# skitzoid/Box2D-MT

Hardware: AMD Instinct MI355X
Metric: world steps/sec at 99858 bodies per GPU (BASELINE config 3: Tumbler 100k, CCD off; Step = collide + island solve + broad-phase + state read-back); for N > 1: container-steps/s = world steps/s x N containers in the one sharded world (higher is better)
Workload: dtype f32

## Files before the change

box2d-mt_amd/csrc/b2d_kernels_collide.h:

```cpp
#ifndef B2D_KERNELS_COLLIDE_H
#define B2D_KERNELS_COLLIDE_H

#include "b2d_world.h"
#include "b2d_toi.h"
#include "b2d_scan.h"

__device__ __forceinline__ Xf loadXf(const float4* b_xf, int body)
{
	float4 t = b_xf[body];
	Xf xf;
	xf.p = v2(t.x, t.y);
	xf.q.s = t.z;
	xf.q.c = t.w;
	return xf;
}

__device__ __forceinline__ AABB loadAabb(const float4* p_fat, int proxy)
{
	float4 t = p_fat[proxy];
	AABB a;
	a.lo = v2(t.x, t.y);
	a.hi = v2(t.z, t.w);
	return a;
}
// ... 390 lines not shown
		c.cellExtBits = 0;
		c.gridFresh = 0;
		W.st->dbgCensus[0] = 0;
		c.nEvents = 0;
		c.nToiList = 0;
		c.nNewToiCand = 0;
		c.nToiEvents = 0;
		c.nToiCalls = 0;
		c.toiBase = 0;
		c.toiOverflow = 0;
		c.nToiLog = 0;
		c.toiIncomplete = 0;
		c.toiUnsafe = 0;
		c.nToiGroups = 0;
		c.nToiMoved = 0;
		c.nToiNewPairs = 0;
		c.nToiChainCreated = 0;
		c.nPreSolve = 0;
		c.nPostSolve = 0;
		c.nFilterList = 0;
		c.spToiCreated = 0;
		c.spToiStraddle = 0;
	}
	if (t < 32) bar[t] = t == 6 ? W.testSpinMax : 0;
	for (int k = t; k < ARRIVE_SITES * TREE_WORDS; k += (int)blockDim.x) W.arriveTree[k] = 0ull;
}

__global__ __launch_bounds__(256) void k_wake_apply(DW W)
{
	b2dPhaseStamp(W);
	for (int i = blockIdx.x * blockDim.x + threadIdx.x; i < W.nBodies; i += gridDim.x * blockDim.x)
	{
		if (W.b_wake[i])
		{
			W.b_flags[i] |= BF_AWAKE;
			W.b_pos[i].w = 0.0f;
			W.b_wake[i] = 0;
		}
	}
}

__global__ __launch_bounds__(256) void k_flag_filter(DW W, const unsigned long long* pairs, int nPairs)
{
	b2dPhaseStamp(W);
	DState* S = W.st;
	const int n = S->c.nContacts;
// ... 198 lines not shown
```

box2d-mt_amd/csrc/b2d_kernels_solve_large.h:

```cpp
#ifndef B2D_KERNELS_SOLVE_LARGE_H
#define B2D_KERNELS_SOLVE_LARGE_H

#include "b2d_kernels_solve_small.h"

#define LC_WORDS ((int)(sizeof(ContactConstraint) / 4))
#define LC_VEL_WORDS 36
#define LC_IMP_FIRST 10
#define LC_MASS_FIRST 28
#define LC_POS_FIRST 36

__device__ __forceinline__ void lcStore(const DW& W, int row, const ContactConstraint& cc, int first, int last)
{
	uint32_t words[LC_WORDS];
	memcpy(words, &cc, sizeof(ContactConstraint));
	uint32_t* dst = (uint32_t*)W.lc;
#pragma unroll
	for (int f = 0; f < LC_WORDS; ++f)
	{
		if (f >= first && f < last) dst[(size_t)f * W.capContacts + row] = words[f];
	}
}

__device__ __forceinline__ void lcLoad(const DW& W, int row, ContactConstraint& cc, int first, int last)
{
// ... 1622 lines not shown
			W.b_vel[body] = make_float4(vv.x, vv.y, w, 0.0f);
		}
	}
	{
		const int n = S->c.nLIslands;
		for (int k = blockIdx.x * blockDim.x + threadIdx.x; k < n; k += gridDim.x * blockDim.x)
		{
			W.rootPen[W.li_roots[k]] = 0;
			W.rootJointOkay[W.li_roots[k]] = 1;
		}
	}
	if (blockIdx.x == 0 && threadIdx.x == 0) S->c.allLargeDone = 0;
}

__global__ __launch_bounds__(256) void k_large_position(DW W, int color)
{
	asm volatile("" :: "s"(W.capContacts), "s"(color), "s"((unsigned long long)(uintptr_t)W.colorStart), "s"((unsigned long long)(uintptr_t)W.st),
		"s"((unsigned long long)(uintptr_t)W.li_ref), "s"((unsigned long long)(uintptr_t)W.lc), "s"((unsigned long long)(uintptr_t)W.b_pos),
		"s"((unsigned long long)(uintptr_t)W.rootDone), "s"((unsigned long long)(uintptr_t)W.rootPen), "s"((unsigned)blockDim.x), "s"((unsigned)gridDim.x), "s"(W.stampMask));
	b2dPhaseStamp(W);
	DState* S = W.st;
	const int allDone = S->c.allLargeDone;
	const int begin = W.colorStart[color], end = W.colorStart[color + 1];
	if (allDone) return;
	const ContactArrays& C = W.ca[S->cur];
	BlockMaxU32 pen;
	pen.key = -1; pen.val = 0u;
	for (int base = begin + blockIdx.x * blockDim.x; base < end; base += gridDim.x * blockDim.x)
	{
		const int row = base + threadIdx.x;
		bool valid = row < end;
		LargeRef r;
		r.root = 0;
		if (valid)
		{
			r = largeRef(W, C, row);
			valid = W.rootDone[r.root] == 0;
		}
		float minSep = 0.0f;
		if (valid)
		{
			ContactConstraint cc;
			memset(&cc, 0, sizeof(cc));
			lcLoad(W, row, cc, LC_MASS_FIRST, LC_MASS_FIRST + 4);
			lcLoad(W, row, cc, LC_POS_FIRST, LC_WORDS);
			float4 pa = W.b_pos[r.bodyA], pb = W.b_pos[r.bodyB];
			BodyPos pA, pB;
			pA.c = v2(pa.x, pa.y); pA.a = pa.z;
			pB.c = v2(pb.x, pb.y); pB.a = pb.z;
			b2dSolvePosition(&cc, &pA, &pB, B2D_BAUMGARTE, &minSep);
			if (r.nsA) W.b_pos[r.bodyA] = make_float4(pA.c.x, pA.c.y, pA.a, pa.w);
			if (r.nsB) W.b_pos[r.bodyB] = make_float4(pB.c.x, pB.c.y, pB.a, pb.w);
		}
		blockMaxU32Offer(pen, W.rootPen, r.root, floatBits(0.0f - minSep), valid);
	}
	blockMaxU32Flush(pen, W.rootPen);
}

__global__ __launch_bounds__(256) void k_large_pos_end(DW W)
{
	b2dPhaseStamp(W);
	DState* S = W.st;
	if (S->c.allLargeDone) return;
	__shared__ int s_open;
	if (threadIdx.x == 0) s_open = 0;
	__syncthreads();
	const int n = S->c.nLIslands;
	int open = 0;
	for (int k = threadIdx.x; k < n; k += blockDim.x)
// ... 85 lines not shown
```

box2d-mt_amd/csrc/b2d_kernels_sweep_end.h:

```cpp
#ifndef B2D_KERNELS_SWEEP_END_H
#define B2D_KERNELS_SWEEP_END_H

#include "b2d_handover.h"

#define SWEEP_END_LANES 512
#define SWEEP_END_WAVES (SWEEP_END_LANES / 64)
#define SE_HUB 1
#define SE_GUESS 2
#define SE_JOINTS_INIT 4
#define SE_JOINTS_VEL 8
#define SE_JOINTS_POS 16
#define SE_POS_END 32
#define SE_POS_BEGIN 64
#define SE_HUB_WIDE_ONLY 128

#define REST_ROWS_MAX 196608
#define REST_SERIAL_BIT (1ull << HUB_COLOR)
template <int MODE>
__device__ __forceinline__ bool restSweepRows(const DW& W, int restFirst, int nColors, int* bar, int epoch, int wg, int nWG, bool serialTagged)
{
	DState* S = W.st;
	const ContactArrays& C = W.ca[S->cur];
	const int begin = W.colorStart[restFirst], end = W.colorStart[nColors];
	const int tag = (epoch & 0x7fff) << 16;
// ... 628 lines not shown
	}
}

__global__ __launch_bounds__(256) void k_solver_recover_reset(DW W, int* bar)
{
	b2dPhaseStamp(W);
	DState* S = W.st;
	for (int i = blockIdx.x * blockDim.x + threadIdx.x; i < W.nBodies; i += gridDim.x * blockDim.x)
	{
		for (int k = 0; k < ROOT_PEN_SLOTS; ++k) W.rootPen[(size_t)k * W.nBodies + i] = 0;
		W.rootDone[i] = 0;
		W.rootSleepMin[i] = 0x7f7fffffu;
		W.rootJointOkay[i] = 1;
		W.bodyRest[i] = 0;
		W.bodyActive[i] = 0;
	}
	for (int i = blockIdx.x * blockDim.x + threadIdx.x; i < MAX_BLOCKS + 1; i += gridDim.x * blockDim.x)
	{
		W.blkCursor[(size_t)i * BLK_SLOT] = 0;
		W.blkBodyCursor[(size_t)i * BLK_SLOT] = 0;
	}
	if (blockIdx.x == 0 && threadIdx.x <= MAX_COLORS) W.colorCursor[colorSlot(threadIdx.x)] = 0;
	if (blockIdx.x == 0 && threadIdx.x < 32) bar[threadIdx.x] = 0;
	if (blockIdx.x == 0 && threadIdx.x == 0)
	{
		atomicAnd(&S->c.overflow, ~(64 | 0x2000));
		S->c.allLargeDone = 0;
		S->c.posItersLarge = 0;
	}
}

#endif
```

box2d-mt_amd/csrc/b2d_world.h:

```cpp
#ifndef B2D_WORLD_H
#define B2D_WORLD_H

#include "b2d_solver.h"
#include "b2d_joint.h"
#include "b2d_wave.h"

#define BF_TYPE_MASK 0x3u
#define BF_AWAKE 0x4u
#define BF_AUTOSLEEP 0x8u
#define BF_BULLET 0x10u
#define BF_FIXEDROT 0x20u
#define BF_ACTIVE 0x40u
#define BF_ISLAND 0x80u
#define BF_LARGE 0x100u

#define BT_STATIC 0u
#define BT_KINEMATIC 1u
#define BT_DYNAMIC 2u

#define CF_TOUCHING 0x1u
#define CF_ENABLED 0x2u
#define CF_FILTER 0x4u
#define CF_TOI_CANDIDATE 0x8u
#define CF_SENSOR 0x10u
// ... 438 lines not shown
{
	if (c.nBlocks == 0 || c.nOrphanRows > 0 || c.blkMaxRows > c.blkLanes || c.blkMaxBodies > c.blkLanes || c.nSerialOrphans > 2048) return false;
	if (c.partitionAge > 240 && (4 * c.nCutRows > c.nLContacts || 2 * c.nLContacts < 900)) return false;
	return true;
}

__device__ __forceinline__ void b2dStoreAgentI(int* p, int v) { __hip_atomic_store(p, v, __ATOMIC_RELAXED, __HIP_MEMORY_SCOPE_AGENT); }
__device__ __forceinline__ int b2dLoadAgentI(const int* p) { return __hip_atomic_load(p, __ATOMIC_RELAXED, __HIP_MEMORY_SCOPE_AGENT); }
__device__ __forceinline__ void b2dStoreAgent4(float4* p, float4 v)
{
	typedef float f4 __attribute__((ext_vector_type(4)));
	f4 q;
	q.x = v.x; q.y = v.y; q.z = v.z; q.w = v.w;
	asm volatile("global_store_dwordx4 %0, %1, off sc1\n\ts_nop 1" :: "v"(p), "v"(q) : "memory");
}
__device__ __forceinline__ float4 b2dLoadAgent4(const float4* p)
{
	typedef float f4 __attribute__((ext_vector_type(4)));
	f4 r;
	asm volatile("global_load_dwordx4 %0, %1, off sc1\n\ts_waitcnt vmcnt(0)" : "=v"(r) : "v"(p) : "memory");
	return make_float4(r.x, r.y, r.z, r.w);
}
#define TREE_GROUPS 32
#define TREE_STRIDE 16
#define TREE_WORDS ((TREE_GROUPS + 1) * TREE_STRIDE)
#define TREE_SUM_MAX 0xffffffu
#define ARRIVE_COLLIDE 0
#define ARRIVE_COMPACT 1
#define ARRIVE_EDGES 2
#define ARRIVE_CHAINS 3
#define ARRIVE_END_STEP 4
#define ARRIVE_CLASSIFY 5
#define ARRIVE_TOI_FIRST 6
#define ARRIVE_COLOR_CHECK 7
#define ARRIVE_PAIRS 8
#define ARRIVE_KEYSET 9
#define ARRIVE_SITES 10
__device__ __forceinline__ bool b2dTreeArrive(unsigned long long* tree, unsigned v0, unsigned v1, unsigned* t0, unsigned* t1)
{
	const unsigned nb = gridDim.x;
	const unsigned groups = nb < TREE_GROUPS ? nb : TREE_GROUPS;
	const unsigned g = blockIdx.x % groups;
	const unsigned members = nb / groups + (g < nb % groups ? 1u : 0u);
	const unsigned long long one = 1ull << 48;
	unsigned long long* slot = tree + (size_t)g * TREE_STRIDE;
	const unsigned long long add = one | ((unsigned long long)(v1 & TREE_SUM_MAX) << 24) | (unsigned long long)(v0 & TREE_SUM_MAX);
// ... 95 lines not shown
```

box2d-mt_amd/csrc/b2hip.hip:

```cpp
#include <hip/hip_runtime.h>

#include <math.h>
#include <stdio.h>
#include <stdlib.h>
#include <string.h>

#include <algorithm>
#include <dlfcn.h>
#include <rccl/rccl.h>
#include <atomic>
#include <chrono>
#include <thread>
#include <map>
#include <mutex>
#include <string>
#include <vector>

#include "../../include/b2hip.h"
#include "b2d_kernels_toi_chains.h"
#include "b2d_kernels_toi_domains.h"
#include "b2d_handover.h"
#include "b2d_kernels_solve_blocks.h"
#include "b2d_kernels_sweep_end.h"
#include "b2d_kernels_edit.h"
#include "b2d_kernels_shard.h"
#include "b2d_kernels_spatial.h"
#include "b2d_kernels_query.h"
#include "b2d_scan.h"
#include "b2d_shape_geom.h"

#include "b2hip_host_world.h"
#include "b2hip_host_phases.h"
#include "b2hip_host_toi.h"

extern "C"
{
#include "b2hip_api_world.h"
#include "b2hip_api_step.h"
#include "b2hip_api_snapshot.h"
#include "b2hip_api_sharding.h"
#include "b2hip_api_callbacks.h"
#include "b2hip_api_query.h"
}
```

box2d-mt_amd/csrc/b2hip_api_world.h:

```cpp


const char* b2hip_last_error(void)
{
	return g_lastError.c_str();
}

const char* b2hip_version(void)
{
	return "b2hip 0.1 (gfx950)";
}

int b2hip_world_create(const b2hip_world_def* def, b2hip_world** out)
{
	if (!def || !out) return setError(B2HIP_ERR_INVALID, "null argument");
	int count = 0;
	hipError_t e = hipGetDeviceCount(&count);
	if (e != hipSuccess || count <= 0)
	{
		return setError(B2HIP_ERR_NO_DEVICE, "no HIP device available: the b2hip Step() path has no CPU fallback");
	}
	int current = 0;
	if (hipGetDevice(&current) != hipSuccess) current = 0;
	const int device = def->device >= 0 ? def->device : current;
	if (device >= count) return setError(B2HIP_ERR_NO_DEVICE, "no such HIP device");
// ... 59 lines not shown
				hipOccupancyMaxActiveBlocksPerMultiprocessor(&perCU2, k_solve_blocks<512>, 512, 0) == hipSuccess &&
				hipOccupancyMaxActiveBlocksPerMultiprocessor(&perCU3, k_solve_blocks<BLOCK_LANES>, BLOCK_LANES, 0) == hipSuccess &&
				perCU > 0 && perCU2 > 0 && perCU3 > 0)
			{
				w->blocksMaxWG = prop.multiProcessorCount - 8;
				int s0 = 0, s1 = 0, s2 = 0;
				if (hipOccupancyMaxActiveBlocksPerMultiprocessor(&s0, k_blocks_sweep<256>, 256, 0) == hipSuccess &&
					hipOccupancyMaxActiveBlocksPerMultiprocessor(&s1, k_blocks_sweep<512>, 512, 0) == hipSuccess &&
					hipOccupancyMaxActiveBlocksPerMultiprocessor(&s2, k_blocks_sweep<BLOCK_LANES>, BLOCK_LANES, 0) == hipSuccess)
				{
					w->sweepMaxWG[0] = std::max(1, s0 - 1) * w->blocksMaxWG;
					w->sweepMaxWG[1] = std::max(1, s1 - 1) * w->blocksMaxWG;
					w->sweepMaxWG[2] = std::max(1, s2 - 1) * w->blocksMaxWG;
				}
			}
			int r1 = 0, r2 = 0, f1 = 0, f2 = 0;
			const int cus = std::max(1, prop.multiProcessorCount - 8);
			if (hipOccupancyMaxActiveBlocksPerMultiprocessor(&r1, k_large_rest<1>, 256, 0) == hipSuccess &&
				hipOccupancyMaxActiveBlocksPerMultiprocessor(&r2, k_large_rest<2>, 256, 0) == hipSuccess && r1 > 0 && r2 > 0)
				w->restMaxWG = std::min(r1, r2) * cus;
			if (hipOccupancyMaxActiveBlocksPerMultiprocessor(&f1, k_rest_hub<1>, SWEEP_END_LANES, 0) == hipSuccess &&
				hipOccupancyMaxActiveBlocksPerMultiprocessor(&f2, k_rest_hub<2>, SWEEP_END_LANES, 0) == hipSuccess && f1 > 0 && f2 > 0)
				w->restHubMaxWG = std::min(f1, f2) * cus;
		}
	}
	w->dfEpoch = 0;
	for (int i = 0; i < 13; ++i) w->ev[i] = nullptr;
	w->h_dstate = nullptr;
	for (int i = 0; i < 13; ++i)
	{
		if (hipEventCreate(&w->ev[i]) != hipSuccess)
		{
			b2hip_world_destroy(w);
			return setError(B2HIP_ERR_HIP, "hipEventCreate failed");
		}
	}
	if (hipHostMalloc((void**)&w->h_dstate, sizeof(DState), hipHostMallocDefault) != hipSuccess)
	{
		b2hip_world_destroy(w);
		return setError(B2HIP_ERR_HIP, "hipHostMalloc failed");
	}
	if (hipHostMalloc((void**)&w->h_pub, sizeof(DState), hipHostMallocMapped | hipHostMallocCoherent) != hipSuccess ||
		hipHostGetDevicePointer((void**)&w->d_pub, w->h_pub, 0) != hipSuccess)
	{
		b2hip_world_destroy(w);
		return setError(B2HIP_ERR_HIP, "hipHostMalloc (coherent) failed");
// ... 697 lines not shown
	StepParams& sp = w->sp;
	sp.dt = dt;
	sp.inv_dt = dt > 0.0f ? 1.0f / dt : 0.0f;
	sp.dtRatio = w->inv_dt0 * dt;
	sp.velIters = velocity_iterations;
	sp.posIters = position_iterations;
	sp.warmStarting = w->def.warm_starting;
	sp.allowSleep = w->def.allow_sleep;
	sp.gravity = v2(w->def.gravity_x, w->def.gravity_y);
	if (w->kernelTiming > 1)
	{
		w->ktUsed = 0;
		w->ktKind = 0;
	}
	w->stepActive = true;
	w->stepSolves = w->stepComplete;
	w->dw.toiContinue = w->stepComplete ? 0 : 1;
	w->dw.toiEventCap = w->def.sub_stepping ? 1 : 0;
	Counters zero;
	memset(&zero, 0, sizeof(zero));
	w->dw.stampMask = 1u << 14;
	LAUNCH(w, k_step_begin, 1, 64, w->dw, w->gridBar.p);
	w->restArrived = 0;
	w->toiStep.countersFresh = true;
	rc = applyPendingFilters(w);
	if (rc) return rc;
	rc = applyEditOps(w, false);
	if (rc) return rc;
	if (w->spatial)
	{
		if (listenerOn(w) || hasFilter(w) || w->def.sub_stepping) return setError(B2HIP_ERR_UNSUPPORTED, "contact listeners, filters and sub-stepping are not supported in a spatially sharded world");
		rc = spBeginStep(w);
		if (rc) return rc;
	}
	stampPhase(w, 0);
	if (w->newFixture)
	{
		rc = findNewContacts(w, true);
		if (rc) return rc;
		w->newFixture = false;
	}
	stampPhase(w, 1);
	return 0;
}

static int checkBody(b2hip_world* w, int body, const char* what)
// ... 538 lines not shown
```

box2d-mt_amd/csrc/b2hip_host_phases.h:

```cpp

static int spExchangeState(b2hip_world* w, int mode);
static int spExchangePairs(b2hip_world* w, long long* totalPairs, int* straddling);
static int spResolve(b2hip_world* w, int nVirt = 0);
static int spAfterToi(b2hip_world* w);
static int spBeginStep(b2hip_world* w);

static int radixBits(int maxKey)
{
	int bits = 1;
	while ((1 << bits) <= maxKey && bits < 31) ++bits;
	return bits;
}

static void radixPasses(int first, int bits, std::vector<std::pair<int, int>>& out)
{
	const int passes = (bits + RADIX_BITS - 1) / RADIX_BITS;
	for (int p = 0, at = 0; p < passes; ++p)
	{
		const int width = (bits - at + (passes - p) - 1) / (passes - p);
		out.push_back(std::make_pair(first + at, width));
		at += width;
	}
}

// ... 641 lines not shown
	if ((w->dfEpoch >> 14) == w->dfWipedAt) return 0;
	HIP_TRY(hipMemsetAsync(w->b_cutv.p, 0, w->b_cutv.cap * sizeof(float4), w->stream));
	HIP_TRY(hipMemsetAsync(w->b_posv.p, 0, w->b_posv.cap * sizeof(float4), w->stream));
	w->dfWipedAt = w->dfEpoch >> 14;
	return 0;
}

struct LargePlan
{
	bool safe = false;
	bool useSweepEnd = false;
	int restFirst = 0x7fffffff;
	long long restRows = 0;
	bool useRest = false;
	int tailFirst = 0;
	bool tailAny = false;
	int bigEnd = 0;
	bool leftoverApart = false;
	bool fuseHub = false;
	bool bodyWarm = false;
	bool hubBuildOne = false;
	bool sortInIntegrate = false;
	bool afterFused = false;
	bool censusGrid = false;
	uint64_t colorMask = ~0ull;
	int gB = 0, gC = 0, gJ = 0;
	int gK = 0;
	bool waitsBetweenWorkgroups = false;
};

static inline bool colorUsed(const LargePlan& p, int col) { return col >= 64 || ((p.colorMask >> col) & 1ull) != 0; }

static LargePlan planLargePass(const b2hip_world* w, const SolveStep& s, const bool safe)
{
	const DW& d = w->dw;
	const StepParams& sp = w->sp;
	const Counters& c = s.c;
	const int nColors = s.nColors;
	LargePlan p;
	p.safe = safe;
	p.gB = gridFor(s.nLBodies);
	p.gC = gridFor(std::max(s.nLContacts, 1));
	p.gJ = gridFor(std::max(s.nLIslands, 1), 64, 1 << 16);
	p.useSweepEnd = w->sweepEnd && !s.exactLarge && !w->debugTrace;
	if (p.useSweepEnd && w->restFlow && !safe && !d.blockSort && !c.needRecolor && !s.censusVoid && nColors > 0 && nColors < MAX_COLORS)
	{
		long long sum = 0;
		int t = nColors;
		while (t > 0 && sum + c.colorRows[t - 1] <= (long long)w->restRowsMax)
		{
			sum += c.colorRows[t - 1];
			t -= 1;
		}
		if (nColors - t >= 2) p.restFirst = t;
// ... 3 lines not shown
	p.useRest = p.useSweepEnd && p.restFirst < nColors;
	p.hubBuildOne = s.hasHubs && !w->noHubBuild && w->last.nHubRows <= HUB_BUILD_LDS;
	p.gK = gridFor(std::max(s.nLContacts / std::max(nColors, 1), 1) * 2);
	p.censusGrid = !s.exactLarge && nColors > 0 && nColors <= MAX_COLORS && !c.needRecolor && !s.censusVoid;
	p.waitsBetweenWorkgroups = s.useBlocks || s.useSweep || p.useRest;
	p.sortInIntegrate = s.hasJoints && !s.exactLarge && !w->debugTrace;
	p.bodyWarm = w->bodyWarm && w->sweepEnd && !s.exactLarge && !w->debugTrace && !s.useSweep && sp.warmStarting && nColors <= MAX_COLORS;
	p.colorMask = s.exactLarge ? ~0ull : ((uint64_t)w->h_dstate->c.colorMaskLo | ((uint64_t)w->h_dstate->c.colorMaskHi << 32));
	p.tailFirst = p.useRest ? p.restFirst : nColors;
	if (p.useSweepEnd && w->sweepTail && !p.useRest && !s.useSweep && !c.needRecolor && !s.censusVoid && nColors <= MAX_COLORS)
	{
		long long sum = 0;
		while (p.tailFirst > 0 && c.colorRows[p.tailFirst - 1] <= w->tailRowsMax && sum + c.colorRows[p.tailFirst - 1] <= 8ll * w->tailRowsMax)
		{
			sum += c.colorRows[p.tailFirst - 1];
			p.tailFirst -= 1;
		}
	}
	for (int col = p.tailFirst; col < nColors && !p.useRest; ++col) p.tailAny = p.tailAny || colorUsed(p, col);
	p.bigEnd = s.useSweep ? 0 : p.tailFirst;
	p.leftoverApart = p.useSweepEnd && s.hasHubs && d.hubWide && c.nHubRows - c.nHubWide > SE_LEFT_INLINE_MAX;
	p.fuseHub = p.useRest && w->restHub && (s.hasHubs || s.hasJoints) && !p.leftoverApart && w->restHubMaxWG > 1;
	p.afterFused = !w->debugTrace && sp.posIters > 0;
	return p;
}

static inline int gridOfColor(const SolveStep& s, const LargePlan& p, int col)
{
	if (!p.censusGrid || col < 0 || col >= MAX_COLORS) return p.gK;
	return gridFor((size_t)s.c.colorRows[col] + 512, 256, 1 << 16);
}

struct LargePass
{
	b2hip_world* const w;
	SolveStep& s;
	const LargePlan p;
	DW& d;
	const StepParams& sp;
	LargePass(b2hip_world* w_, SolveStep& s_, bool safe) : w(w_), s(s_), p(planLargePass(w_, s_, safe)), d(w_->dw), sp(w_->sp) {}

	template <typename Launch>
	int withEpoch(Launch launch)
	{
		if (int rc = wipeHandoverRows(w)) return rc;
		if (int rc = launch()) return rc;
		w->dfEpoch += 1;
		return 0;
	}

	static const int WHOLE_SOLVE = -1;
	int launchBlocks(int mode)
	{
		const Counters& c = s.c;
// ... 81 lines not shown
	}

	int setUp()
	{
		TRACE("before_integrate");
		if (w->debugTrace)
		{
			const size_t nb = w->bodies.size();
			(void)w->dbgPreVel.ensure(nb, w->stream); (void)w->dbgVel.ensure(nb, w->stream); (void)w->dbgLi.ensure(nb + 64, w->stream);
			HIP_TRY(hipMemcpyAsync(w->dbgPreVel.p, w->b_vel.p, nb * 16, hipMemcpyDeviceToDevice, w->stream));
			HIP_TRY(hipMemcpyAsync(w->dbgLi.p, w->li_bodies.p, nb * 4, hipMemcpyDeviceToDevice, w->stream));
			HIP_TRY(hipMemcpyAsync(w->dbgLi.p + nb, &w->d_state.p->c, 64 * 4 > sizeof(Counters) ? sizeof(Counters) : 64 * 4, hipMemcpyDeviceToDevice, w->stream));
		}
		if (w->kernelTiming == 5 && !p.safe) { int rc = ktRecord(w); if (rc) return rc; w->ktKind = 8; w->familyLaunchesAtStart = w->launchCount; }
		LAUNCH(w, k_large_integrate, p.gB, 256, d, sp, p.sortInIntegrate ? 1 : 0);
		if (w->debugTrace) HIP_TRY(hipMemcpyAsync(w->dbgVel.p, w->b_vel.p, w->bodies.size() * 16, hipMemcpyDeviceToDevice, w->stream));
		TRACE("integrate");
		if (s.hasJoints && !s.exactLarge && !p.sortInIntegrate) LAUNCH(w, k_joints_sort, p.gJ, 64, d);
		LAUNCH(w, k_large_init, p.gC, 256, d, sp, p.bodyWarm ? 1 : 0);
		TRACE("init");
		return 0;
	}

	int sweepColours(int mode, int it)
	{
		if (s.useSweep) return launchBlocks(mode);
		const bool timeIt = mode == 1 && w->kernelTiming == 1;
		for (int col = 0; col < p.bigEnd; ++col)
		{
			if (!colorUsed(p, col)) continue;
			if (timeIt) { int rc = ktRecord(w); if (rc) return rc; w->ktKind = 1; }
			if (mode == 2) LAUNCH(w, k_large_position, gridOfColor(s, p, col), 256, d, col);
			else LAUNCH(w, k_large_velocity, gridOfColor(s, p, col), 256, d, col, mode);
			if (timeIt) { int rc = ktRecord(w); if (rc) return rc; }
			if (mode > 0 && w->debugTrace) TRACE(((mode == 1 ? "vel" : "pos") + std::to_string(it) + "_c" + std::to_string(col)).c_str());
		}
		return 0;
	}

	int whatFollows(int mode, int it) const
	{
		int what = s.hasHubs ? SE_HUB | (it > 0 ? SE_GUESS : 0) : 0;
		if (mode == 0 && s.hasJoints) what |= SE_JOINTS_INIT | (sp.velIters > 0 ? SE_JOINTS_VEL : 0);
		if (mode == 1 && s.hasJoints && it + 1 < sp.velIters) what |= SE_JOINTS_VEL;
		if (mode == 2) what |= (s.hasJoints ? SE_JOINTS_POS : 0) | SE_POS_END | (it + 1 < sp.posIters ? SE_POS_BEGIN : 0);
		return what;
	}

	int endOfSweep(int mode, int it, bool coloursDone = false)
// ... 79 lines not shown
		}
		if (rc) return rc;
		LAUNCH(w, k_large_finalize, p.gB, 256, d, sp);
		TRACE("finalize");
		LAUNCH(w, k_large_sleep, p.gB, 256, d, sp);
		return 0;
	}
};

static int recoverLarge(b2hip_world* w, SolveStep& s)
{
	DW& d = w->dw;
	w->solverSeq = (w->solverSeq + 1) & 0x7fff;
	LAUNCH(w, k_solver_status, 1, 64, d, w->d_solverWord, w->solverSeq);
	if (int rc = pollPublished(w, (volatile const int*)&w->h_solverWord[1], w->solverSeq, "solver status")) return rc;
	const int flags = w->h_solverWord[0];
	const bool colorsBad = s.colorsOnDevice && ((flags & 4) != 0 || w->h_solverWord[2] != 0);
	if (s.colorsOnDevice) w->colorSmallPending = false;
	if (!(flags & 64) && !colorsBad) return 0;
	if (w->tracePartition || w->traceRecovery) fprintf(stderr, "[b2hip] a wait between workgroups of the large-island solver timed out (overflow 0x%x): saved state back, the solve once more launch by launch\n", flags);
	LAUNCH(w, k_solver_snapshot, gridFor(std::max(s.nLBodies, s.nLContacts)), 256, d, 1);
	LAUNCH(w, k_solver_recover_reset, gridFor(d.nBodies), 256, d, w->gridBar.p);
	w->restArrived = 0;
	if (int rc = readState(w)) return rc;
	if (colorsBad)
	{
		if (w->traceRecovery) fprintf(stderr, "[b2hip] the resident solver ran on an incomplete colouring (overflow 0x%x, %d without a colour): colouring finished, the solve once more\n", flags, w->h_solverWord[2]);
		if (int rc = colorRoundsUntilDone(w, s, w->h_dstate->c.nUncolored, 8)) return rc;
		if (w->h_dstate->c.overflow & 4) s.colorSpill = s.hasHubs = true;
		s.censusVoid = true;
		w->colorRecoveries += 1;
	}
	s.nColors = std::min(w->h_dstate->c.nColors, (int)HUB_COLOR);
	s.c.nColors = s.nColors;
	memcpy(s.c.colorRows, w->h_dstate->c.colorRows, sizeof(s.c.colorRows));
	if (flags & 64) w->solverRecoveries += 1;
	s.useBlocks = s.useSweep = false;
	s.colorsOnDevice = false;
	d.blockSort = 0;
	return LargePass(w, s, true).run();
}

static int solveLargeIslands(b2hip_world* w, SolveStep& s)
{
	if (!s.exactLarge) s.nColors = s.c.nColors;
	s.hasJoints = w->dw.nJoints > 0;
// ... 257 lines not shown
```

box2d-mt_amd/csrc/b2hip_host_world.h:

```cpp

static thread_local std::string g_lastError;

static int setError(int code, const std::string& msg)
{
	g_lastError = msg;
	return code;
}

#define HIP_TRY(expr)                                                                                   \
	do                                                                                                  \
	{                                                                                                   \
		hipError_t _e = (expr);                                                                         \
		if (_e != hipSuccess)                                                                           \
		{                                                                                               \
			return setError(B2HIP_ERR_HIP, std::string(#expr) + ": " + hipGetErrorString(_e));          \
		}                                                                                               \
	} while (0)

static void (*g_rcclDestroy)(void* comm) = nullptr;

template <typename T>
struct DevArray
{
	T* p = nullptr;
// ... 311 lines not shown
	bool sweepTail = true;
	int tailRowsMax = 1024;
	int freshColors = 0;
	bool freshColorsPending = false;
	bool forceOnDevice = true;
	int rowMarks = 1;
	bool rowsWentEarly = false;
	bool sweepStamps = false;
	bool bodyWarm = true;
	bool restFlow = true;
	bool noHubBuild = false;
	bool noHubOrder = false;
	bool hubOrderAll = false;
	bool recoverOn = true;
	int* h_solverWord = nullptr;
	int* d_solverWord = nullptr;
	int solverSeq = 0;
	int colorRecoveries = 0;
	int solverRecoveries = 0;
	int sweepRowsMax = 60000;
	int restHub = 2;
	int restHubMaxWG = 0;
	int restMaxWG = 0;
	int restArrived = 0;
	int restRowsMax = 65536;
	long long launchCount = 0;
	long long familyLaunchesAtStart = 0; int familyLaunches = 0;
	int largeHintSteps = 120;
	int serialOrphansNext = 0;
	int adoptSticky = 0;
	bool adoptPasses = false;
	bool traceLaunches = false;
	bool tracePartition = false;
	bool traceRecovery = false;
	bool handoverWhy = false;
	bool shardTrace = false;
	double stepDeadlineS = 300.0;
	int pollDelayUs = 0;
	bool gridHalf = false;
	bool gridForced = false;
	int pairsLargeSticky = 0;
	int recolorCountdown = 0;
	bool blocksTooBig = false;
	bool noSweepBlocks = false;
	int dfWipedAt = 0;
	int sweepSteps = 0;
// ... 439 lines not shown
	w->recoverOn = !envOn("B2HIP_NO_RECOVER");
	w->noCensusPoll = envOn("B2HIP_NO_CENSUS_POLL");
	w->noStatePoll = envOn("B2HIP_NO_STATE_POLL");
	w->lazyReadback = envOn("B2HIP_LAZY_READBACK");
	w->earlyRowsMin = envInt("B2HIP_EARLY_ROWS_MIN", w->earlyRowsMin);
	w->stepDeadlineS = getenv("B2HIP_STEP_DEADLINE_S") ? atof(getenv("B2HIP_STEP_DEADLINE_S")) : 300.0;
	w->pollDelayUs = envInt("B2HIP_TEST_POLL_DELAY_US", 0);
	d.bigChunks = envSet("B2HIP_BIG_CHUNKS") ? 1 : 0;
	d.smallMaxW = TINY_ISLAND_MAX_W;
	if (const char* e = getenv("B2HIP_SMALL_MAX_W")) d.smallMaxW = std::max(1, std::min((int)SMALL_ISLAND_MAX_W, atoi(e)));
	d.noFreeBodies = envOn("B2HIP_NO_FREE_BODIES") ? 1 : 0;
	d.testMaxColors = envInt("B2HIP_TEST_MAX_COLORS", 0);
	d.testColorRounds = envInt("B2HIP_TEST_COLOR_ROUNDS", 0);
	d.testSpinMax = std::max(0, envInt("B2HIP_TEST_SPIN_MAX", 0));
	d.restPoll = getenv("B2HIP_REST_POLL") ? std::max(1, std::min(16, atoi(getenv("B2HIP_REST_POLL")))) : 1;
	d.hubSerial = envOn("B2HIP_HUB_SERIAL") ? 1 : 0;
	w->hubWaves = envInt("B2HIP_HUB_WAVES", 0) == 1 ? 1 : 8;
	w->sweepEnd = !envOn("B2HIP_NO_SWEEP_END") && !envSet("B2HIP_HUB_WAVES");
	w->sweepTail = w->sweepEnd && !envOn("B2HIP_NO_TAIL");
	w->sweepStamps = envSet("B2HIP_SWEEP_STAMPS");
	w->rowMarks = envOn("B2HIP_ROW_MARKS_CHECK") ? 2 : envOn("B2HIP_NO_ROW_MARKS") ? 0 : 1;
	w->bodyWarm = !envOn("B2HIP_NO_BODY_WARM");
	w->restFlow = w->sweepEnd && !envOn("B2HIP_NO_REST");
	w->noHubBuild = envOn("B2HIP_NO_HUB_BUILD");
	w->noHubOrder = envOn("B2HIP_NO_HUB_ORDER");
	w->hubOrderAll = envOn("B2HIP_HUB_ORDER");
	if (getenv("B2HIP_SWEEP_ROWS_MAX")) w->sweepRowsMax = std::max(1, atoi(getenv("B2HIP_SWEEP_ROWS_MAX")));
	w->restHub = getenv("B2HIP_REST_HUB") ? std::max(0, std::min(2, atoi(getenv("B2HIP_REST_HUB")))) : 2;
	w->restRowsMax = getenv("B2HIP_REST_ROWS") ? std::min(atoi(getenv("B2HIP_REST_ROWS")), REST_ROWS_MAX - COLOR_SMALL_MAX) : 65536;
	w->tailRowsMax = envInt("B2HIP_TAIL_ROWS", SWEEP_END_LANES);
	d.hubWide = (w->sweepEnd && !d.hubSerial && envInt("B2HIP_HUB_WIDE", 1) != 0) ? 1 : 0;
}

static int ensureCapacity(b2hip_world* w, size_t needContacts)
{
	hipStream_t s = w->stream;
	const size_t nb = std::max<size_t>(w->bodies.size(), 1);
	const size_t np = std::max<size_t>(w->fixtures.size(), 1);
	int rc = 0;
#define ENS(arr, n) do { rc = w->arr.ensure((n), s); if (rc) return rc; } while (0)
	ENS(d_state, 1);
	ENS(b_pos, nb); ENS(b_pos0, nb); ENS(b_vel, nb); ENS(b_xf, nb); ENS(b_mass, nb); ENS(b_damp, nb); ENS(b_force, nb);
	ENS(b_flags, nb); ENS(b_wake, nb); ENS(b_rowDirty, nb); ENS(b_order, nb); ENS(orderBody, nb); ENS(bigRoots, SHARD_BIG_MAX);
	ENS(p_fat, np); ENS(p_body, np); ENS(p_shape, np); ENS(p_key, np); ENS(p_filter0, np); ENS(p_filter1, np); ENS(p_mat, np);
	ENS(b_proxyHead, nb); ENS(p_next, np);
	ENS(d_shapes, std::max<size_t>(w->shapes.size(), 1));
// ... 63 lines not shown
	if (w->collideCompactOn)
	{
		const size_t chunks = cc / (size_t)w->collideChunk + 2;
		rc = w->collideCounts.ensure(chunks, s, false); if (rc) return rc;
		rc = w->collideGroups.ensure(chunks / COLLIDE_GROUP + 2, s, false); if (rc) return rc;
	}
	ENS(toiList, cc); ENS(toiPos2c, cc); ENS(toiDestroyList, cc); ENS(toiNewList, TOI_NEW_LIST_MAX);
	ENS(b_toiGroup, nb); ENS(toiGroups, nb); ENS(toiGroupCount, std::min<size_t>(nb, TOI_GROUPS_MAX)); ENS(toiGroupList, std::min<size_t>(nb, TOI_GROUPS_MAX) * CHAIN_ADJ_MAX); ENS(toiMoved, TOI_MOVED_ALL_MAX); ENS(toiNew, 8 * TOI_NEWPAIR_MAX); ENS(toiParent, nb); ENS(toiDomOf, nb); ENS(toiDomRoot, TOI_DOMAINS_MAX); ENS(toiDomCount, TOI_DOMAINS_MAX); ENS(toiDomBase, TOI_DOMAINS_MAX); ENS(toiDomFill, TOI_DOMAINS_MAX); ENS(toiDomFailed, TOI_DOMAINS_MAX); ENS(toiDomEvents, TOI_DOMAINS_MAX); ENS(toiDomList, cc); ENS(toiHull, np); ENS(snapBody, 5 * nb); ENS(snapFat, np);
	{
		const size_t nPre = hasPreSolve(w) ? cc : 1, nPost = w->postSolveOn ? cc : 1, nFil = hasFilter(w) ? cc : 1;
		ENS(pre_o0, nPre); ENS(pre_o1, nPre); ENS(pre_oimp, nPre); ENS(pre_o3, nPre); ENS(preRecs, nPre);
		ENS(postRecs, nPost); ENS(filterList, nFil);
		ENS(toiLog, listenerOn(w) && w->def.continuous ? cc : 1);
		ENS(toiVerdict, hasPreSolve(w) && w->def.continuous ? cc : 1);
		ENS(hostList, std::max<size_t>(std::max(4 * nPre, nFil), hasFilter(w) ? capPairs : 1));
	}
	ENS(b_blk1, nb); ENS(b_adopt, nb); ENS(b_adoptStage, 3 * nb); ENS(blkRows, (size_t)(MAX_BLOCKS + 2) * BLK_SLOT); ENS(blkRowStart, MAX_BLOCKS + 2); ENS(blkCursor, (size_t)(MAX_BLOCKS + 2) * BLK_SLOT); ENS(blkBodyCount, (size_t)(MAX_BLOCKS + 2) * BLK_SLOT); ENS(blkBodyCursor, (size_t)(MAX_BLOCKS + 2) * BLK_SLOT);
	ENS(blkBodyStart, MAX_BLOCKS + 2); ENS(blkBodies, nb); ENS(rowColor, cc); ENS(b_cutv, nb);
	ENS(b_owner, w->spatial ? nb : 1); ENS(spNewOwner, w->spatial ? nb : 1); ENS(spAwake, w->spatial ? nb : 1); ENS(spStraddle, w->spatial ? std::max<size_t>(w->spStraddle.cap, 4096) : 1);
	ENS(spCount, w->spatial ? (size_t)SP_RESOLVE_MAX * SHARD_MAX_RANKS : 1); ENS(spTarget, w->spatial ? SP_RESOLVE_MAX : 1);
	ENS(spTailKey, w->spatial ? capContacts : 1); ENS(spVirt, w->spatial ? SP_TAIL_MAX + 1 : 1);
	ENS(stateOut, 12 * nb + sizeof(DState) / sizeof(float) + 4);
	ENS(consts, 16);
	ENS(gridBar, 32);
#undef ENS
	w->scanCtx.words = w->scanFlags.p;
	w->scanCtx.count = w->scanFlags.cap;
	w->scanCtx.abortWord = &w->d_state.p->c.overflow;
	w->radixCtx.counts = w->radixCounts.p; w->radixCtx.countsCap = w->radixCounts.cap;
	w->radixCtx.groups = w->radixGroups.p; w->radixCtx.groupsCap = w->radixGroups.cap;
	w->radixCtx.hist = w->radixGlobalHist.p;
	w->radixCtx.maxTiles = w->sortOnepass ? (int)std::min<size_t>(std::min<size_t>(w->radixCounts.cap / RADIX_DIGITS, (w->radixGroups.cap / RADIX_DIGITS) * RADIX_GROUP), RADIX_ONEPASS_MAX_TILES) : 0;
	w->radixCtx.abortWord = &w->d_state.p->c.overflow;
	if (w->h_stateCap < 12 * nb + sizeof(DState) / sizeof(float) + 4)
	{
		ensureRows(w);
		float* old = w->h_state;
		w->h_state = nullptr;
		w->h_stateCap = 12 * nb * 2 + sizeof(DState) / sizeof(float) + 4;
		HIP_TRY(hipHostMalloc((void**)&w->h_state, w->h_stateCap * sizeof(float), hipHostMallocMapped | hipHostMallocCoherent));
		HIP_TRY(hipHostGetDevicePointer((void**)&w->d_hstate, w->h_state, 0));
		if (old)
		{
			memcpy(w->h_state, old, w->stateCount * 10 * sizeof(float));
			(void)hipHostFree(old);
		}
	}
// ... 403 lines not shown
```

Baseline: 375.0.

## Fuse per-colour solver launches into one persistent kernel with grid barriers

Adds a persistent k_colour_sweep kernel that walks every used graph colour in a single launch and separates colours with a slotted atomic grid barrier, where it previously issued one kernel launch per colour. While one colour is being solved it prefetches the next colour's constraint rows. It is meant to cut per-colour launch overhead and the idle time between dependent kernels. The grid is capped at one workgroup per CU so all blocks stay co-resident, and spinning on global atomics risks stalls. k_large_position is also changed to issue its loads before the allDone and rootDone checks.

After: 369.3. 0.985x the previous value.

```diff
diff --git a/box2d-mt_amd/csrc/b2d_kernels_collide.h b/box2d-mt_amd/csrc/b2d_kernels_collide.h
--- a/box2d-mt_amd/csrc/b2d_kernels_collide.h
+++ b/box2d-mt_amd/csrc/b2d_kernels_collide.h
@@ -436,6 +436,7 @@
 		c.spToiCreated = 0;
 		c.spToiStraddle = 0;
 	}
+	for (int k = t; k < CS_SLOTS; k += (int)blockDim.x) bar[CS_BAR_FIRST + k * CS_SLOT_INTS] = 0;
 	if (t < 32) bar[t] = t == 6 ? W.testSpinMax : 0;
 	for (int k = t; k < ARRIVE_SITES * TREE_WORDS; k += (int)blockDim.x) W.arriveTree[k] = 0ull;
 }
diff --git a/box2d-mt_amd/csrc/b2d_kernels_colour_sweep.h b/box2d-mt_amd/csrc/b2d_kernels_colour_sweep.h
--- /dev/null
+++ b/box2d-mt_amd/csrc/b2d_kernels_colour_sweep.h
@@ -0,0 +1,222 @@
+#ifndef B2D_KERNELS_COLOUR_SWEEP_H
+#define B2D_KERNELS_COLOUR_SWEEP_H
+
+#include "b2d_kernels_sweep_end.h"
+
+
+__device__ __forceinline__ bool colourBarrier(int* bar, int* overflow, int need, int spinMax, bool stamped, unsigned long long& tDrained, unsigned long long& tJoined, unsigned long long& tPolled)
+{
+	__shared__ int s_ok;
+	asm volatile("s_waitcnt vmcnt(0)" ::: "memory");
+	if (stamped) tDrained = wall_clock64();
+	__syncthreads();
+	if (stamped) tJoined = wall_clock64();
+	if (threadIdx.x < 64u)
+	{
+		const int lane = (int)threadIdx.x;
+		if (lane == 0) (void)__hip_atomic_fetch_add(&bar[CS_BAR_FIRST + (int)(blockIdx.x & (CS_SLOTS - 1)) * CS_SLOT_INTS], 1, __ATOMIC_RELAXED, __HIP_MEMORY_SCOPE_AGENT);
+		const int* const mine = lane < CS_SLOTS ? &bar[CS_BAR_FIRST + lane * CS_SLOT_INTS] : &bar[4];
+		int ok = 1, spins = 0;
+		auto weigh = [&](int v) -> int
+		{
+			const int aborted = __shfl(v, CS_SLOTS);
+			int sum = lane < CS_SLOTS ? v : 0;
+#pragma unroll
+			for (int off = CS_SLOTS / 2; off > 0; off >>= 1) sum += __shfl_xor(sum, off);
+			sum = __shfl(sum, 0);
+			if (aborted != 0) return 2;
+			if (sum - need >= 0) return 1;
+			if (++spins > spinMax)
+			{
+				if (lane == 0) { stcI(&bar[4], 1); atomicOr(overflow, 64); }
+				return 2;
+			}
+			return 0;
+		};
+		int v0 = ldcI(mine), v1 = 0, verdict = 0;
+		for (;;)
+		{
+			v1 = ldcI(mine);
+			if ((verdict = weigh(v0)) != 0) break;
+			__builtin_amdgcn_s_sleep(1);
+			v0 = ldcI(mine);
+			if ((verdict = weigh(v1)) != 0) break;
+			__builtin_amdgcn_s_sleep(1);
+		}
+		ok = verdict == 1 ? 1 : 0;
+		if (lane == 0) s_ok = ok;
+		if (stamped) tPolled = wall_clock64();
+	}
+	__syncthreads();
+	return s_ok != 0;
+}
+
+struct ColourRow
+{
+	int row;
+	bool have;
+	bool open;
+	int4 ref;
+	LargeRef r;
+	ContactConstraint cc;
+};
+
+template <int MODE>
+__device__ __forceinline__ void colourRowFetch(const DW& W, const ContactArrays& C, int row, bool have, ColourRow& q)
+{
+	const int at = have ? row : 0;
+	(void)C;
+	q.row = row;
+	q.have = have;
+	q.open = have;
+	memset(&q.cc, 0, sizeof(q.cc));
+	q.r.ci = 0; q.r.bodyA = 0; q.r.bodyB = 0; q.r.root = 0; q.r.nsA = false; q.r.nsB = false;
+	q.ref = W.li_ref[at];
+	if (MODE == 2)
+	{
+		lcLoad(W, at, q.cc, LC_MASS_FIRST, LC_MASS_FIRST + 4);
+		lcLoad(W, at, q.cc, LC_POS_FIRST, LC_WORDS);
+	}
+	else lcLoad(W, at, q.cc, 0, LC_VEL_WORDS);
+}
+
+__device__ __forceinline__ void colourRowOpen(const DW& W, ColourRow& q)
+{
+	q.open = W.rootDone[q.ref.w] == 0 && q.have;
+}
+
+template <int MODE>
+__device__ __forceinline__ void colourRowBodies(const DW& W, ColourRow& q, float4& a, float4& b)
+{
+	q.r.ci = q.ref.x;
+	q.r.nsA = q.ref.y >= 0;
+	q.r.nsB = q.ref.z >= 0;
+	q.r.bodyA = q.r.nsA ? q.ref.y : -(q.ref.y + 1);
+	q.r.bodyB = q.r.nsB ? q.ref.z : -(q.ref.z + 1);
+	q.r.root = q.ref.w;
+	const float4* const rows = MODE == 2 ? W.b_pos : W.b_vel;
+	f4v ra, rb;
+	ldRow2(&rows[q.r.bodyA], &rows[q.r.bodyB], &ra, &rb);
+	a = make_float4(ra.x, ra.y, ra.z, ra.w);
+	b = make_float4(rb.x, rb.y, rb.z, rb.w);
+	if (MODE != 2)
+	{
+		if (!q.r.nsA) a = make_float4(0, 0, 0, 0);
+		if (!q.r.nsB) b = make_float4(0, 0, 0, 0);
+	}
+}
+
+__device__ __forceinline__ void colourRowStore(float4* p, const float4 v)
+{
+	stRow(p, v.x, v.y, v.z, __float_as_int(v.w));
+}
+
+template <int MODE>
+__device__ __forceinline__ void colourRowSolve(const DW& W, ColourRow& q, const float4 a, const float4 b, BlockMaxU32& pen)
+{
+	if (MODE == 2)
+	{
+		float minSep = 0.0f;
+		if (q.open)
+		{
+			BodyPos pA, pB;
+			pA.c = v2(a.x, a.y); pA.a = a.z;
+			pB.c = v2(b.x, b.y); pB.a = b.z;
+			b2dSolvePosition(&q.cc, &pA, &pB, B2D_BAUMGARTE, &minSep);
+			if (q.r.nsA) colourRowStore(&W.b_pos[q.r.bodyA], make_float4(pA.c.x, pA.c.y, pA.a, a.w));
+			if (q.r.nsB) colourRowStore(&W.b_pos[q.r.bodyB], make_float4(pB.c.x, pB.c.y, pB.a, b.w));
+		}
+		blockMaxU32Offer(pen, W.rootPen, q.r.root, floatBits(0.0f - minSep), q.open);
+	}
+	else if (q.have)
+	{
+		BodyVel vA, vB;
+		vA.v = v2(a.x, a.y); vA.w = a.z;
+		vB.v = v2(b.x, b.y); vB.w = b.z;
+		b2dSolveVelocity(&q.cc, &vA, &vB);
+		lcStore(W, q.row, q.cc, LC_IMP_FIRST, LC_IMP_FIRST + 4);
+		if (q.r.nsA) colourRowStore(&W.b_vel[q.r.bodyA], make_float4(vA.v.x, vA.v.y, vA.w, 0.0f));
+		if (q.r.nsB) colourRowStore(&W.b_vel[q.r.bodyB], make_float4(vB.v.x, vB.v.y, vB.w, 0.0f));
+	}
+}
+
+template <int MODE>
+__global__ __launch_bounds__(256) void k_colour_sweep(DW W, unsigned long long mask, int bigEnd, int* bar, int base, int* stampBar)
+{
+	asm volatile("" :: "s"(W.capContacts), "s"((unsigned)(mask & 0xffffffffull)), "s"((unsigned)(mask >> 32)), "s"(bigEnd), "s"(base),
+		"s"((unsigned long long)(uintptr_t)bar), "s"((unsigned long long)(uintptr_t)stampBar), "s"((unsigned long long)(uintptr_t)W.colorStart),
+		"s"((unsigned long long)(uintptr_t)W.st), "s"((unsigned long long)(uintptr_t)W.li_ref), "s"((unsigned long long)(uintptr_t)W.lc),
+		"s"((unsigned long long)(uintptr_t)W.b_vel), "s"((unsigned long long)(uintptr_t)W.b_pos), "s"((unsigned long long)(uintptr_t)W.rootDone),
+		"s"((unsigned long long)(uintptr_t)W.rootPen), "s"((unsigned)gridDim.x), "s"(W.stampMask));
+	b2dPhaseStamp(W);
+	DState* S = W.st;
+	const unsigned long long t0 = stampBar != nullptr ? wall_clock64() : 0ull;
+	const int allDone = MODE == 2 ? S->c.allLargeDone : 0;
+	const int spinLimit = bar[6];
+	unsigned long long todo = mask & (bigEnd >= 64 ? ~0ull : ((1ull << bigEnd) - 1ull));
+	if (todo == 0ull) return;
+	__shared__ int s_start[MAX_COLORS + 1];
+	if ((int)threadIdx.x <= bigEnd && threadIdx.x <= MAX_COLORS) s_start[threadIdx.x] = W.colorStart[threadIdx.x];
+	const int nWG = (int)gridDim.x;
+	if (allDone)
+	{
+		const int nBar = __popcll(todo) - 1;
+		if (threadIdx.x == 0 && nBar > 0) (void)__hip_atomic_fetch_add(&bar[CS_BAR_FIRST + (int)(blockIdx.x & (CS_SLOTS - 1)) * CS_SLOT_INTS], nBar, __ATOMIC_RELAXED, __HIP_MEMORY_SCOPE_AGENT);
+		return;
+	}
+	__syncthreads();
+	const ContactArrays& C = W.ca[S->cur];
+	const int spinMax = spinLimit != 0 ? spinLimit : PERSIST_SPIN_MAX;
+	const int mine = (int)(blockIdx.x * 256u + threadIdx.x), stride = nWG * 256;
+	BlockMaxU32 pen;
+	pen.key = -1; pen.val = 0u;
+	int need = base;
+	int col = __ffsll((long long)todo) - 1;
+	int begin = s_start[col], end = s_start[col + 1];
+	const bool prof = MODE == 1 && stampBar != nullptr && blockIdx.x == 0;
+	unsigned long long tDrained = 0ull, tJoined = 0ull, tPolled = 0ull, tTop = t0;
+	int acc0 = 0, acc1 = 0, acc2 = 0, acc3 = 0, acc4 = 0, acc5 = 0;
+	ColourRow next;
+	colourRowFetch<MODE>(W, C, begin + mine, begin + mine < end, next);
+	if (MODE == 2) colourRowOpen(W, next);
+	for (;;)
+	{
+		todo &= todo - 1ull;
+		ColourRow cur = next;
+		const int curBegin = begin, curEnd = end;
+		float4 rowA, rowB;
+		if (prof) tTop = wall_clock64();
+		colourRowBodies<MODE>(W, cur, rowA, rowB);
+		const unsigned long long tBodies = prof ? wall_clock64() : 0ull;
+		const bool last = todo == 0ull;
+		if (!last) col = __ffsll((long long)todo) - 1;
+		begin = s_start[col]; end = s_start[col + 1];
+		colourRowFetch<MODE>(W, C, begin + mine, begin + mine < end, next);
+		colourRowSolve<MODE>(W, cur, rowA, rowB, pen);
+		if (MODE == 2) colourRowOpen(W, next);
+		for (int b = curBegin + stride; b < curEnd; b += stride)
+		{
+			colourRowFetch<MODE>(W, C, b + mine, b + mine < curEnd, cur);
+			if (MODE == 2) colourRowOpen(W, cur);
+			colourRowBodies<MODE>(W, cur, rowA, rowB);
+			colourRowSolve<MODE>(W, cur, rowA, rowB, pen);
+		}
+		if (last) break;
+		need += nWG;
+		const unsigned long long tSolved = prof ? wall_clock64() : 0ull;
+		if (!colourBarrier(bar, &S->c.overflow, need, spinMax, prof, tDrained, tJoined, tPolled)) return;
+		if (prof)
+		{
+			acc0 += (int)(tBodies - tTop); acc1 += (int)(tSolved - tBodies); acc2 += (int)(tDrained - tSolved);
+			acc3 += (int)(tJoined - tDrained); acc4 += (int)(tPolled - tJoined); acc5 += (int)(wall_clock64() - tPolled);
+		}
+	}
+	if (prof && threadIdx.x == 0)
+	{
+		stampBar[14] = acc0; stampBar[15] = acc1; stampBar[16] = acc2; stampBar[17] = acc3; stampBar[18] = acc4; stampBar[19] = acc5;
+	}
+	if (MODE == 2) blockMaxU32Flush(pen, W.rootPen);
+	if (stampBar != nullptr && blockIdx.x == 0 && threadIdx.x == 0) stampBar[MODE == 2 ? 13 : 12] = (int)(wall_clock64() - t0);
+}
+
+#endif
diff --git a/box2d-mt_amd/csrc/b2d_kernels_solve_large.h b/box2d-mt_amd/csrc/b2d_kernels_solve_large.h
--- a/box2d-mt_amd/csrc/b2d_kernels_solve_large.h
+++ b/box2d-mt_amd/csrc/b2d_kernels_solve_large.h
@@ -1668,7 +1668,6 @@
 	DState* S = W.st;
 	const int allDone = S->c.allLargeDone;
 	const int begin = W.colorStart[color], end = W.colorStart[color + 1];
-	if (allDone) return;
 	const ContactArrays& C = W.ca[S->cur];
 	BlockMaxU32 pen;
 	pen.key = -1; pen.val = 0u;
@@ -1677,20 +1676,23 @@
 		const int row = base + threadIdx.x;
 		bool valid = row < end;
 		LargeRef r;
-		r.root = 0;
+		r.ci = 0; r.bodyA = 0; r.bodyB = 0; r.root = 0; r.nsA = false; r.nsB = false;
+		ContactConstraint cc;
+		memset(&cc, 0, sizeof(cc));
+		float4 pa = make_float4(0, 0, 0, 0), pb = pa;
 		if (valid)
 		{
 			r = largeRef(W, C, row);
-			valid = W.rootDone[r.root] == 0;
-		}
+			lcLoad(W, row, cc, LC_MASS_FIRST, LC_MASS_FIRST + 4);
+			lcLoad(W, row, cc, LC_POS_FIRST, LC_WORDS);
+			const int done = W.rootDone[r.root];
+			pa = W.b_pos[r.bodyA]; pb = W.b_pos[r.bodyB];
+			valid = done == 0;
+		}
+		if (allDone) return;
 		float minSep = 0.0f;
 		if (valid)
 		{
-			ContactConstraint cc;
-			memset(&cc, 0, sizeof(cc));
-			lcLoad(W, row, cc, LC_MASS_FIRST, LC_MASS_FIRST + 4);
-			lcLoad(W, row, cc, LC_POS_FIRST, LC_WORDS);
-			float4 pa = W.b_pos[r.bodyA], pb = W.b_pos[r.bodyB];
 			BodyPos pA, pB;
 			pA.c = v2(pa.x, pa.y); pA.a = pa.z;
 			pB.c = v2(pb.x, pb.y); pB.a = pb.z;
diff --git a/box2d-mt_amd/csrc/b2d_kernels_sweep_end.h b/box2d-mt_amd/csrc/b2d_kernels_sweep_end.h
--- a/box2d-mt_amd/csrc/b2d_kernels_sweep_end.h
+++ b/box2d-mt_amd/csrc/b2d_kernels_sweep_end.h
@@ -674,6 +674,7 @@
 	}
 	if (blockIdx.x == 0 && threadIdx.x <= MAX_COLORS) W.colorCursor[colorSlot(threadIdx.x)] = 0;
 	if (blockIdx.x == 0 && threadIdx.x < 32) bar[threadIdx.x] = 0;
+	if (blockIdx.x == 0 && threadIdx.x < CS_SLOTS) bar[CS_BAR_FIRST + threadIdx.x * CS_SLOT_INTS] = 0;
 	if (blockIdx.x == 0 && threadIdx.x == 0)
 	{
 		atomicAnd(&S->c.overflow, ~(64 | 0x2000));
diff --git a/box2d-mt_amd/csrc/b2d_world.h b/box2d-mt_amd/csrc/b2d_world.h
--- a/box2d-mt_amd/csrc/b2d_world.h
+++ b/box2d-mt_amd/csrc/b2d_world.h
@@ -484,6 +484,10 @@
 	return make_float4(r.x, r.y, r.z, r.w);
 }
 #define TREE_GROUPS 32
+#define CS_SLOTS 32
+#define CS_SLOT_INTS 32
+#define CS_BAR_FIRST 32
+#define CS_BAR_INTS (CS_BAR_FIRST + CS_SLOTS * CS_SLOT_INTS)
 #define TREE_STRIDE 16
 #define TREE_WORDS ((TREE_GROUPS + 1) * TREE_STRIDE)
 #define TREE_SUM_MAX 0xffffffu
diff --git a/box2d-mt_amd/csrc/b2hip.hip b/box2d-mt_amd/csrc/b2hip.hip
--- a/box2d-mt_amd/csrc/b2hip.hip
+++ b/box2d-mt_amd/csrc/b2hip.hip
@@ -22,6 +22,7 @@
 #include "b2d_handover.h"
 #include "b2d_kernels_solve_blocks.h"
 #include "b2d_kernels_sweep_end.h"
+#include "b2d_kernels_colour_sweep.h"
 #include "b2d_kernels_edit.h"
 #include "b2d_kernels_shard.h"
 #include "b2d_kernels_spatial.h"
diff --git a/box2d-mt_amd/csrc/b2hip_api_world.h b/box2d-mt_amd/csrc/b2hip_api_world.h
--- a/box2d-mt_amd/csrc/b2hip_api_world.h
+++ b/box2d-mt_amd/csrc/b2hip_api_world.h
@@ -105,6 +105,10 @@
 			if (hipOccupancyMaxActiveBlocksPerMultiprocessor(&f1, k_rest_hub<1>, SWEEP_END_LANES, 0) == hipSuccess &&
 				hipOccupancyMaxActiveBlocksPerMultiprocessor(&f2, k_rest_hub<2>, SWEEP_END_LANES, 0) == hipSuccess && f1 > 0 && f2 > 0)
 				w->restHubMaxWG = std::min(f1, f2) * cus;
+			int c1 = 0, c2 = 0;
+			if (hipOccupancyMaxActiveBlocksPerMultiprocessor(&c1, k_colour_sweep<1>, 256, 0) == hipSuccess &&
+				hipOccupancyMaxActiveBlocksPerMultiprocessor(&c2, k_colour_sweep<2>, 256, 0) == hipSuccess && c1 > 0 && c2 > 0)
+				w->colourSweepMaxWG = cus;
 		}
 	}
 	w->dfEpoch = 0;
@@ -848,6 +852,7 @@
 	w->dw.stampMask = 1u << 14;
 	LAUNCH(w, k_step_begin, 1, 64, w->dw, w->gridBar.p);
 	w->restArrived = 0;
+	w->colourArrived = 0;
 	w->toiStep.countersFresh = true;
 	rc = applyPendingFilters(w);
 	if (rc) return rc;
diff --git a/box2d-mt_amd/csrc/b2hip_host_phases.h b/box2d-mt_amd/csrc/b2hip_host_phases.h
--- a/box2d-mt_amd/csrc/b2hip_host_phases.h
+++ b/box2d-mt_amd/csrc/b2hip_host_phases.h
@@ -687,6 +687,9 @@
 	bool hubBuildOne = false;
 	bool sortInIntegrate = false;
 	bool afterFused = false;
+	bool colourSweep = false;
+	int gSweep = 0;
+	int sweepBarriers = 0;
 	bool censusGrid = false;
 	uint64_t colorMask = ~0ull;
 	int gB = 0, gC = 0, gJ = 0;
@@ -695,6 +698,12 @@
 };
 
 static inline bool colorUsed(const LargePlan& p, int col) { return col >= 64 || ((p.colorMask >> col) & 1ull) != 0; }
+
+static inline int gridOfColor(const SolveStep& s, const LargePlan& p, int col)
+{
+	if (!p.censusGrid || col < 0 || col >= MAX_COLORS) return p.gK;
+	return gridFor((size_t)s.c.colorRows[col] + 512, 256, 1 << 16);
+}
 
 static LargePlan planLargePass(const b2hip_world* w, const SolveStep& s, const bool safe)
 {
@@ -744,14 +753,25 @@
 	p.leftoverApart = p.useSweepEnd && s.hasHubs && d.hubWide && c.nHubRows - c.nHubWide > SE_LEFT_INLINE_MAX;
 	p.fuseHub = p.useRest && w->restHub && (s.hasHubs || s.hasJoints) && !p.leftoverApart && w->restHubMaxWG > 1;
 	p.afterFused = !w->debugTrace && sp.posIters > 0;
+	if (w->colourSweep && p.censusGrid && !safe && !s.useSweep && !s.useBlocks && !w->debugTrace && w->kernelTiming != 1 && w->colourSweepMaxWG > 0)
+	{
+		int used = 0, g = 1;
+		for (int col = 0; col < p.bigEnd; ++col)
+		{
+			if (!colorUsed(p, col)) continue;
+			used += 1;
+			g = std::max(g, gridOfColor(s, p, col));
+		}
+		g = std::min(g, w->colourSweepMaxWG);
+		if (w->colourSweepTestGrid > 0) g = std::min(g, w->colourSweepTestGrid);
+		p.colourSweep = used >= 2;
+		p.gSweep = g;
+		p.sweepBarriers = used - 1;
+		p.waitsBetweenWorkgroups = p.waitsBetweenWorkgroups || p.colourSweep;
+	}
 	return p;
 }
 
-static inline int gridOfColor(const SolveStep& s, const LargePlan& p, int col)
-{
-	if (!p.censusGrid || col < 0 || col >= MAX_COLORS) return p.gK;
-	return gridFor((size_t)s.c.colorRows[col] + 512, 256, 1 << 16);
-}
 
 struct LargePass
 {
@@ -879,9 +899,19 @@
 		return 0;
 	}
 
+	int launchColourSweep(int mode)
+	{
+		int* const stamps = w->sweepStamps ? w->gridBar.p : (int*)nullptr;
+		if (mode == 1) LAUNCH(w, k_colour_sweep<1>, p.gSweep, 256, d, p.colorMask, p.bigEnd, w->gridBar.p, w->colourArrived, stamps);
+		else LAUNCH(w, k_colour_sweep<2>, p.gSweep, 256, d, p.colorMask, p.bigEnd, w->gridBar.p, w->colourArrived, stamps);
+		w->colourArrived += p.gSweep * p.sweepBarriers;
+		return 0;
+	}
+
 	int sweepColours(int mode, int it)
 	{
 		if (s.useSweep) return launchBlocks(mode);
+		if (p.colourSweep && mode != 0) return launchColourSweep(mode);
 		const bool timeIt = mode == 1 && w->kernelTiming == 1;
 		for (int col = 0; col < p.bigEnd; ++col)
 		{
@@ -1007,6 +1037,7 @@
 	LAUNCH(w, k_solver_snapshot, gridFor(std::max(s.nLBodies, s.nLContacts)), 256, d, 1);
 	LAUNCH(w, k_solver_recover_reset, gridFor(d.nBodies), 256, d, w->gridBar.p);
 	w->restArrived = 0;
+	w->colourArrived = 0;
 	if (int rc = readState(w)) return rc;
 	if (colorsBad)
 	{
diff --git a/box2d-mt_amd/csrc/b2hip_host_world.h b/box2d-mt_amd/csrc/b2hip_host_world.h
--- a/box2d-mt_amd/csrc/b2hip_host_world.h
+++ b/box2d-mt_amd/csrc/b2hip_host_world.h
@@ -357,6 +357,10 @@
 	int restHub = 2;
 	int restHubMaxWG = 0;
 	int restMaxWG = 0;
+	bool colourSweep = true;
+	int colourSweepMaxWG = 0;
+	int colourSweepTestGrid = 0;
+	int colourArrived = 0;
 	int restArrived = 0;
 	int restRowsMax = 65536;
 	long long launchCount = 0;
@@ -842,6 +846,8 @@
 	w->rowMarks = envOn("B2HIP_ROW_MARKS_CHECK") ? 2 : envOn("B2HIP_NO_ROW_MARKS") ? 0 : 1;
 	w->bodyWarm = !envOn("B2HIP_NO_BODY_WARM");
 	w->restFlow = w->sweepEnd && !envOn("B2HIP_NO_REST");
+	w->colourSweep = envInt("B2HIP_COLOR_SWEEP", 1) != 0;
+	w->colourSweepTestGrid = std::max(0, envInt("B2HIP_TEST_SWEEP_GRID", 0));
 	w->noHubBuild = envOn("B2HIP_NO_HUB_BUILD");
 	w->noHubOrder = envOn("B2HIP_NO_HUB_ORDER");
 	w->hubOrderAll = envOn("B2HIP_HUB_ORDER");
@@ -951,7 +957,7 @@
 	ENS(spTailKey, w->spatial ? capContacts : 1); ENS(spVirt, w->spatial ? SP_TAIL_MAX + 1 : 1);
 	ENS(stateOut, 12 * nb + sizeof(DState) / sizeof(float) + 4);
 	ENS(consts, 16);
-	ENS(gridBar, 32);
+	ENS(gridBar, CS_BAR_INTS);
 #undef ENS
 	w->scanCtx.words = w->scanFlags.p;
 	w->scanCtx.count = w->scanFlags.cap;
```
